# Bergvca/string_grouper

Hardware: AMD Instinct MI355X
Metric: hot-path rows/sec (the device path of match_strings: tokenise + tf-idf + postings + SpGEMM-topn, inputs resident in HBM), 663k-name self-join ntop=10 min_sim=0.8; match_strings end to end: match_strings_rows_per_s (higher is better)
Workload: dtype f32

## Files before the change

string_grouper_amd/csrc/sg_internal.h:

```cpp
#pragma once

#include <hip/hip_runtime.h>
#include <stdint.h>
#include <stdio.h>
#include <stdlib.h>
#include <string.h>

#include <map>
#include <memory>
#include <mutex>
#include <new>
#include <string>
#include <vector>

#include "../../include/sg_hip.h"

#define SG_WAVE 64
#define SG_NUM_XCD 8

void sg_set_error(const char *fmt, ...);

#define SG_HIP_TRY(expr)                                                                        \
    do {                                                                                        \
        hipError_t _e = (expr);                                                                 \
// ... 202 lines not shown
    int64_t n_orig = 0, n_u = 0;
    uint32_t *d_gid = nullptr;
    uint32_t *d_group_ptr = nullptr;
    uint32_t *d_members = nullptr;
    uint32_t *d_rep_rows = nullptr;
    int64_t *d_rep_start = nullptr;
    int32_t *d_rep_len = nullptr;
    struct sg_csr *unique = nullptr;
    const struct sg_csr *pending_src = nullptr;
};

struct sg_postings {
    sg_ctx *ctx = nullptr;
    int64_t n_right = 0, n_terms = 0, nnz = 0;
    int32_t dtype = SG_F32;
    int32_t tile_log2 = 12;
    int32_t n_tiles = 0;
    const int64_t *b_indptr = nullptr;
    const int32_t *b_indices = nullptr;
    const void *b_data = nullptr;
    uint32_t *d_seg = nullptr;
    uint32_t *d_term_len = nullptr;
    uint32_t *d_term_start = nullptr;
    int32_t *d_rows = nullptr;
    void *d_vals = nullptr;
    sg_csr src;
    int32_t split = 1;
    void *d_fwd = nullptr;
    uint32_t *d_fwd_ptr = nullptr;
    void *d_blk = nullptr;
    uint32_t blk_bytes = 0;
    void *d_q8 = nullptr;
    mutable bool q8_early = true;
    uint32_t *d_filt = nullptr;
    sg_csr *permuted = nullptr;
    uint32_t *d_orig_of = nullptr, *d_pos_of = nullptr;
    struct SgScoreCtx *d_score_ctx = nullptr;
    uint32_t *d_ends = nullptr;
    int32_t nt_pad = 0;
    int32_t fold_log2 = 0;
    uint32_t *d_ends8 = nullptr;
    int32_t nv_pad = 0;
    float norm_up = 0.f;
    uint32_t freq_min = 0;
    bool cosine_like = false;
    float max_norm2 = 0.f;
// ... 128 lines not shown
```

string_grouper_amd/csrc/sg_postings.hip:

```cpp
#include <stdlib.h>

#include <memory>
#include <optional>

#include "sg_internal.h"
#include "sg_scan.h"

__device__ __forceinline__ int64_t row_of_thread(int64_t g, int32_t tile_log2, int32_t n_tiles) {
    return ((g % n_tiles) << tile_log2) | (g / n_tiles);
}

template <typename T>
__global__ void __launch_bounds__(256) postings_count(const int64_t *__restrict__ indptr,
                                                      const int32_t *__restrict__ indices, int64_t n_rows,
                                                      int32_t tile_log2, int32_t n_tiles, uint32_t *seg_counts) {
    const int64_t j = row_of_thread((int64_t)blockIdx.x * blockDim.x + threadIdx.x, tile_log2, n_tiles);
    if (j >= n_rows) return;
    const int64_t lo = indptr[j], hi = indptr[j + 1];
    const uint32_t t = (uint32_t)(j >> tile_log2);
    for (int64_t p = lo; p < hi; ++p) {
        const int64_t bin = (int64_t)indices[p] * n_tiles + t;
        atomicAdd(&seg_counts[bin], 1u);
    }
}
// ... 174 lines not shown
        if (sc_out && threadIdx.x == 0) {
            sc_out[0] = sc;
            sc.q8 = nullptr;
            sc.q8_scale = 0.f;
            sc_out[1] = sc;
        }
        if (null_slack && threadIdx.x < 512) null_slack[threadIdx.x] = sg_null_posting(threadIdx.x);
    }
    const int x = threadIdx.x & 63, y = threadIdx.x >> 6;
    const int64_t k0 = (int64_t)blockIdx.x * 64;
    auto S = [&](int64_t k, int64_t t) -> uint32_t {
        if (k >= n_terms) return term_start[n_terms];
        return t >= n_tiles ? term_start[k + 1] : term_start[k] + cnt[(t * split) * (int64_t)n_terms + k];
    };
    const int64_t t_lim = nt_pad > n_tiles ? nt_pad : n_tiles;
    for (int64_t tb = 0; tb < t_lim; tb += 64) {
        for (int tt = y; tt < 65; tt += 16) {
            const int64_t k = k0 + x;
            tile[x][tt] = k <= n_terms ? S(k, min(tb + tt, (int64_t)n_tiles)) : 0u;
        }
        __syncthreads();
        for (int kq = y; kq < 64; kq += 16) {
            const int64_t k = k0 + kq, t = tb + x;
            if (k < n_terms && t < n_tiles) seg[k * n_tiles + t] = tile[kq][x];
            if (k == n_terms && t == 0) seg[k * n_tiles] = tile[kq][0];
            if (ends && k <= n_terms && t < nt_pad)
                ends[k * nt_pad + t] = k == n_terms ? 0u : tile[kq][min(t, (int64_t)n_tiles - 1) + 1 - tb] << 2;
        }
        __syncthreads();
    }
    if (ends8) {
        for (int64_t i = threadIdx.x; i < (int64_t)64 * nv_pad; i += blockDim.x) {
            const int64_t k = k0 + (i & 63), v = i >> 6;
            if (k > n_terms) continue;
            ends8[k * nv_pad + v] = k == n_terms ? 0u : S(k, min((v + 1) << fold_log2, (int64_t)n_tiles)) << 2;
        }
    }
}

template <typename T>
__global__ void __launch_bounds__(1024) postings_fill_lds(const int64_t *__restrict__ indptr,
                                                          const int32_t *__restrict__ indices,
                                                          const T *__restrict__ data, int64_t n_rows, int32_t tile_log2,
                                                          int32_t n_terms, int32_t split,
                                                          const uint32_t *__restrict__ cnt ,
                                                          const uint32_t *__restrict__ term_start,
                                                          const uint8_t *__restrict__ is_frequent, int32_t *out_rows,
                                                          T *out_vals, uint32_t *out_filt, float inv_norm_up, int32_t fold_log2) {
// ... 305 lines not shown
#pragma unroll
                for (int b = 0; b < FB; ++b) {
                    const uint32_t e = e0 + (uint32_t)b * stride + (uint32_t)lane;
                    const uint64_t heads = __ballot(head[b]) & (~0ull >> (63 - lane));
                    const int src = heads ? 63 - __builtin_clzll(heads) : 0;
                    const uint32_t d = (uint32_t)__shfl((int)delta[b], src, 64);
                    if (e < tot) out_filt[d + e] = stage[e];
                }
            }
        }
        __syncthreads();
        if (!one_chunk) {
            for (uint32_t e = threadIdx.x; e < tot; e += blockDim.x) {
                const uint32_t k = (uint32_t)sterm[e];
                const uint32_t start = k == 0u ? 0u : lds_get16(lcnt, k - 1u);
                if (e == start) mine[k] += lds_get16(lcnt, k) - start;
            }
            __syncthreads();
        }
    }
}

__global__ void __launch_bounds__(256) term_len_kernel(const uint32_t *__restrict__ seg, int64_t n_terms, int32_t n_tiles,
                                                       uint32_t *__restrict__ term_len) {
    const int64_t k = (int64_t)blockIdx.x * blockDim.x + threadIdx.x;
    if (k < n_terms) term_len[k] = seg[(k + 1) * n_tiles] - seg[k * n_tiles];
}

template <typename T>
__global__ void __launch_bounds__(256) fwd_pack(const int64_t *__restrict__ indptr, const int32_t *__restrict__ indices,
                                                const T *__restrict__ data, int64_t n_rows, int64_t nnz,
                                                const uint32_t *__restrict__ orig_of ,
                                                uint32_t *__restrict__ fwd_ptr , void *__restrict__ fwd) {
    const int64_t i = (int64_t)blockIdx.x * blockDim.x + threadIdx.x;
    const int64_t base = indptr[0];
    if (i <= n_rows)
        reinterpret_cast<uint2 *>(fwd_ptr)[i] = make_uint2((uint32_t)(indptr[i] - base), i < n_rows ? (orig_of ? orig_of[i] : (uint32_t)i) : 0u);
    if (i >= nnz || fwd == nullptr) return;
    const int64_t p = base + i;
    if (sizeof(T) == 4) {
        reinterpret_cast<int2 *>(fwd)[i] = make_int2(indices[p], __float_as_int((float)data[p]));
    } else {
        const long long bits = __double_as_longlong((double)data[p]);
        reinterpret_cast<int4 *>(fwd)[i] = make_int4(indices[p], 0, (int)(bits & 0xffffffffll), (int)(bits >> 32));
    }
}

template <typename T>
__global__ void __launch_bounds__(256) row_blocks_kernel(const int64_t *__restrict__ indptr, const int32_t *__restrict__ indices,
// ... 315 lines not shown

static uint32_t q8_rest_unknown(const sg_ctx *ctx) { return ctx->opt_is("SG_Q8_EARLY", '0') ? ~0u : 0u; }
int sg_postings_sync_q8_early(sg_ctx *ctx, const sg_postings *Bt) {
    const bool want = q8_rest_unknown(ctx) == 0u;
    if (!Bt->d_q8 || Bt->q8_early == want || Bt->n_right <= 0) return SG_OK;
    hipLaunchKernelGGL(q8_rest_kernel, dim3((unsigned)((Bt->n_right + 255) / 256)), dim3(256), 0, ctx->stream, (uint4 *)Bt->d_q8,
                       Bt->n_right, want ? 0u : ~0u);
    if (hipGetLastError() != hipSuccess) return SG_ERR_HIP;
    Bt->q8_early = want;
    return SG_OK;
}

static size_t lds_counter_bytes(int64_t n_cols) { return (size_t)n_cols * 4 + ((size_t)(n_cols + 31) / 32) * 4; }

struct BuildPlan {
    bool cosine_like = false;
    float max_norm2 = 0.f;
    int32_t tile_cols = 0, tile_log2 = 0;
    int64_t n_tiles = 0, n_bins = 0;
    bool want_pruned = false, will_filter = false, want_q8 = false, want_blk = false;
    bool permute = false;
    bool early_rows = false;
    bool lds_path = false, lazy_full = false;
    int32_t fold_log2 = 0, nt_pad = 0, nv_pad = 0;
    float norm_up = 0.f;
    uint32_t freq_min = 0;
    bool staged = false;
    int32_t chunk_rows = 0;
    uint32_t stage_cap = 0;
    uint32_t stage_alloc = 0;
    size_t staged_lds = 0;
    int32_t split = 1;
};

struct SplitCost {
    int32_t split = 1;
    int64_t parts = 0, part_rows = 0, chunks = 0, fill_rounds = 0;
    double fill_us = 0, table_us = 0, total_us = 0;
};
static constexpr double SG_SPLIT_US_PER_TERM_AND_CHUNK = 0.78e-3, SG_SPLIT_US_PER_POSTING = 2.9e-3, SG_SPLIT_US_PER_POSTING_RECOUNT = 0.53e-3,
                        SG_SPLIT_US_PER_CELL = 3.7e-6;
static constexpr int32_t SG_SPLIT_MAX = 16, SG_SPLIT_MIN_PART_ROWS = 512;
static SplitCost split_cost(int32_t split, int32_t tile_log2, int64_t n_tiles, int64_t n_terms, double mean_nnz, int32_t chunk_rows,
                            int32_t num_cu) {
    SplitCost c;
    c.split = split;
// ... 59 lines not shown
    pl.n_tiles = B->n_rows == 0 ? 1 : ((B->n_rows + tile_cols - 1) >> pl.tile_log2);
    pl.n_bins = B->n_cols * pl.n_tiles;
    if (pl.n_bins + 1 >= (int64_t)1 << 31) {
        sg_set_error("segment table of %lld x %lld entries is too large; use more right-hand blocks",
                     (long long)B->n_cols, (long long)pl.n_tiles);
        return SG_ERR_OVERFLOW;
    }
    pl.norm_up = __builtin_nextafterf(sqrtf(max_norm2) * 1.000001f, 2.f);
    const bool q8_forced = ctx->opt_is("SG_Q8", '1');
    pl.want_q8 = pl.want_pruned && !(flags & SG_POSTINGS_TILE_FORM) && B->n_cols < ((int64_t)1 << 24) && !ctx->opt_is("SG_Q8", '0') &&
                 (q8_forced || (double)B->nnz <= 45.0 * (double)B->n_rows) &&
                 (ctx->total_mem == 0 || (size_t)SG_Q8_STRIDE * ((size_t)B->n_rows + 1) < ctx->total_mem / 16);
    pl.will_filter = pl.want_pruned && sg_pruned_supports_tile(pl.tile_log2) &&
                     (B->n_cols + 1) * ((pl.n_tiles + 3) & ~(int64_t)3) < ((int64_t)1 << 30);
    pl.want_blk = ctx->opt_is("SG_ROW_BLOCKS", '1');
    pl.permute = !(flags & SG_POSTINGS_NO_PERMUTATION);
    pl.early_rows = pl.will_filter && !pl.want_blk && pl.permute && B->n_rows > 0;
    pl.lds_path = B->n_rows > 0 && lds_counter_bytes(B->n_cols) <= 124 * 1024 && B->n_cols > 0;
    if (const char *e = ctx->opt("SG_POSTINGS_LDS")) pl.lds_path = pl.lds_path && e[0] != '0';
    pl.lazy_full = pl.will_filter && pl.lds_path && !ctx->opt_is("SG_POSTINGS_LAZY", '0');
    if (pl.will_filter) {
        pl.nt_pad = (int32_t)((pl.n_tiles + 3) & ~(int64_t)3);
        if (pl.tile_log2 == 12 && !ctx->opt_is("SG_K4_STREAM", '0')) pl.fold_log2 = 3;
        if (pl.fold_log2 > 0) {
            const int64_t n_super = (pl.n_tiles + ((int64_t)1 << pl.fold_log2) - 1) >> pl.fold_log2;
            pl.nv_pad = (int32_t)((n_super + 3) & ~(int64_t)3);
        }
        double frac = 0.005;
        if (const char *v = ctx->opt("SG_PRUNE_FREQ")) frac = atof(v);
        const double fm = frac * (double)B->n_rows;
        pl.freq_min = fm < 1.0 ? 1u : (uint32_t)fm;
    }
    if (pl.lds_path) {
        pl.staged = pl.lazy_full && !ctx->opt_is("SG_FILL_STAGED", '0') && B->n_cols <= 65535;
        const double mean_nnz = B->n_rows > 0 ? (double)B->nnz / (double)B->n_rows : 1.0;
        if (pl.staged) {
            const size_t fixed0 = ((((size_t)B->n_cols + 1) / 2 + 3) & ~(size_t)3) * 4 + (((size_t)B->n_cols + 31) / 32) * 4 + 32 * 4;
            const size_t room = fixed0 + 16384 < 158 * 1024 ? 158 * 1024 - fixed0 : 0;
            const double per_row = (mean_nnz * 1.2 > 1.0 ? mean_nnz * 1.2 : 1.0) * 6.0 + 4.0;
            const double fit = ((double)room - 64.0 * 6.0 - 32.0) / per_row;
            pl.chunk_rows = fit >= 2048.0 ? 2048 : (fit > 0.0 ? (int32_t)fit & ~63 : 0);
            pl.staged = pl.chunk_rows >= 64;
            const size_t rowp_bytes = (size_t)staged_rowp_words(pl.chunk_rows) * 4;
            pl.stage_alloc = pl.staged ? (uint32_t)((room - rowp_bytes) / 6) & ~1u : 0u;
            if (pl.stage_alloc > 65534u) pl.stage_alloc = 65534u;
            pl.stage_cap = pl.stage_alloc;
// ... 113 lines not shown
        *out = (uint32_t)need;
    return SG_OK;
}

static int alloc_index(sg_ctx *ctx, sg_postings *p, const sg_csr *B_in, const sg_csr *B, const BuildPlan &plan, int32_t flags,
                       Scratch &early, EarlyRows *rows) {
    p->n_right = B->n_rows;
    p->n_terms = B->n_cols;
    p->nnz = B->nnz;
    p->dtype = B->dtype;
    p->tile_log2 = plan.tile_log2;
    p->tile_form = (flags & SG_POSTINGS_TILE_FORM) != 0;
    p->built_from = csr_view(*B_in);
    p->built_from_valid = true;
    p->n_tiles = (int32_t)plan.n_tiles;
    p->b_indptr = B_in->d_indptr;
    p->b_indices = B_in->d_indices;
    p->b_data = B_in->d_data;
    p->cosine_like = plan.cosine_like;
    p->max_norm2 = plan.max_norm2;
    p->src = csr_view(*B);
    p->split = plan.split;
    const size_t vs = 8;
    SG_TRY(sg_alloc(ctx, (size_t)plan.n_bins + 1, &p->d_seg));
    SG_TRY(sg_alloc(ctx, (size_t)B->n_cols + 1, &p->d_term_len));
    if (!plan.lazy_full && B->dtype == SG_F64) SG_TRY(sg_alloc(ctx, (size_t)B->nnz + 64, &p->d_rows));
    if (!plan.lazy_full) SG_TRY(ctx->alloc(((size_t)B->nnz + 64) * vs, &p->d_vals));
    if (!plan.will_filter) return SG_OK;
    if (plan.want_blk) {
        SG_TRY(row_block_bytes(ctx, B, &p->blk_bytes));
        if (p->blk_bytes) SG_TRY(ctx->alloc((size_t)p->blk_bytes * ((size_t)B->n_rows + 1), &p->d_blk));
    }
    p->q8_early = q8_rest_unknown(ctx) == 0u;
    if (rows->written) {
        p->d_fwd = early.keep(rows->fwd);
        p->d_fwd_ptr = early.keep(rows->fwd_ptr);
        p->d_q8 = early.keep(rows->q8);
    } else {
        if (!p->d_blk) SG_TRY(ctx->alloc(((size_t)B->nnz + 8) * (B->dtype == SG_F64 ? 16 : 8), &p->d_fwd));
        SG_TRY(sg_alloc(ctx, 2 * ((size_t)B->n_rows + 2), &p->d_fwd_ptr));
        if (plan.want_q8 && !p->d_blk) SG_TRY(ctx->alloc((size_t)SG_Q8_STRIDE * ((size_t)B->n_rows + 1), &p->d_q8));
    }
    SG_TRY(sg_alloc(ctx, (size_t)B->nnz + 512, &p->d_filt));
    p->nt_pad = plan.nt_pad;
    SG_TRY(sg_alloc(ctx, (size_t)(B->n_cols + 1) * (size_t)p->nt_pad + 4, &p->d_ends));
    p->fold_log2 = plan.fold_log2;
    p->nv_pad = plan.nv_pad;
// ... 24 lines not shown
        SG_TRY(by_dtype(B->dtype, [&](auto tag) -> int {
            using T = decltype(tag);
            constexpr auto kern = postings_fill_lds<T>;
            SG_TRY(allow_dynamic_lds<kern>(124 * 1024));
            hipLaunchKernelGGL(kern, dim3(wgs), dim3(1024), lds, ctx->stream, B->d_indptr, B->d_indices,
                               (const T *)B->d_data, B->n_rows, p->tile_log2, (int32_t)B->n_cols, split, (const uint32_t *)cnt,
                               (const uint32_t *)p->d_term_start, (const uint8_t *)is_frequent, p->d_rows, (T *)p->d_vals, filt,
                               inv_norm, fold_log2);
            return SG_OK;
        }));
    return hipGetLastError() == hipSuccess ? SG_OK : SG_ERR_HIP;
}

static int fill_lds_path(sg_ctx *ctx, sg_postings *p, const BuildPlan &plan) {
    const sg_csr *B = &p->src;
    const unsigned wgs = (unsigned)((int64_t)p->n_tiles * plan.split);
    Scratch scratch(ctx);
    uint32_t *cnt = nullptr, *cnt16 = nullptr;
    uint8_t *is_frequent = nullptr;
    SG_TRY(scratch.alloc((size_t)((int64_t)p->n_tiles * plan.split * B->n_cols) + 1, &cnt));
    if (plan.staged) SG_TRY(scratch.alloc((size_t)((int64_t)p->n_tiles * plan.split * ((B->n_cols + 1) / 2)) + 1, &cnt16));
    SG_TRY(scratch.alloc((size_t)B->n_cols + 4, &is_frequent));
    SG_TRY(sg_alloc(ctx, (size_t)B->n_cols + 2, &p->d_term_start));
    SG_TRY(lds_count_scan_fill(ctx, p, cnt, cnt16, p->d_term_len, is_frequent, false, !plan.staged));
    if (p->d_fwd_ptr) SG_TRY(ctx->alloc(256, (void **)&p->d_score_ctx));
    hipLaunchKernelGGL(postings_tables_kernel, dim3((unsigned)((B->n_cols + 64) / 64)), dim3(1024), 0, ctx->stream, (const uint32_t *)cnt,
                       (const uint32_t *)p->d_term_start, (int32_t)B->n_cols, p->n_tiles, plan.split, p->d_seg, p->d_ends,
                       p->nt_pad, p->d_ends8, p->nv_pad, p->fold_log2, score_ctx_of(p), p->d_score_ctx,
                       p->d_filt ? p->d_filt + B->nnz : (uint32_t *)nullptr);
    if (plan.staged)
        SG_TRY(by_dtype(B->dtype, [&](auto tag) -> int {
            using T = decltype(tag);
            constexpr auto kern = postings_fill_staged<T>;
            SG_TRY(allow_dynamic_lds<kern>(160 * 1024));
            hipLaunchKernelGGL(kern, dim3(wgs), dim3(1024), plan.staged_lds, ctx->stream, B->d_indptr,
                               B->d_indices, (const T *)B->d_data, B->n_rows, p->tile_log2, (int32_t)B->n_cols, plan.split,
                               plan.chunk_rows, plan.stage_cap, plan.stage_alloc, cnt, (const uint32_t *)cnt16,
                               (const uint32_t *)p->d_term_start, (const uint8_t *)is_frequent,
                               p->d_filt, 1.0f / p->norm_up, p->fold_log2);
            return SG_OK;
        }));
    return hipGetLastError() == hipSuccess ? SG_OK : SG_ERR_HIP;
}

static int fill_global_path(sg_ctx *ctx, sg_postings *p, const BuildPlan &plan) {
    const sg_csr *B = &p->src;
// ... 9 lines not shown
        by_dtype(B->dtype, [&](auto tag) {
            using T = decltype(tag);
            hipLaunchKernelGGL(postings_count<T>, dim3(grid), dim3(256), 0, ctx->stream, B->d_indptr, B->d_indices, B->n_rows,
                               p->tile_log2, p->n_tiles, p->d_seg);
            return SG_OK;
        });
        SG_HIP_TRY(hipGetLastError());
    }
    SG_TRY(sg_exclusive_scan_u32(ctx, p->d_seg, p->d_seg, n_bins, p->d_seg + n_bins));
    if (grid > 0) {
        by_dtype(B->dtype, [&](auto tag) {
            using T = decltype(tag);
            hipLaunchKernelGGL(postings_fill<T>, dim3(grid), dim3(256), 0, ctx->stream, B->d_indptr, B->d_indices,
                               (const T *)B->d_data, B->n_rows, p->tile_log2, p->n_tiles, p->d_seg, cursor, p->d_rows,
                               (T *)p->d_vals, p->d_filt, p->freq_min, inv_norm, p->fold_log2);
            return SG_OK;
        });
        if (hipGetLastError() != hipSuccess) return SG_ERR_HIP;
    }
    return SG_OK;
}

static int tables_from_seg(sg_ctx *ctx, sg_postings *p) {
    if (p->n_terms <= 0) return SG_OK;
    hipLaunchKernelGGL(term_len_kernel, dim3((unsigned)((p->n_terms + 255) / 256)), dim3(256), 0, ctx->stream,
                       (const uint32_t *)p->d_seg, p->n_terms, p->n_tiles, p->d_term_len);
    if (p->d_ends || p->d_ends8)
        hipLaunchKernelGGL(ends_from_seg_kernel, dim3((unsigned)((p->n_terms + 256) / 256)), dim3(256), 0, ctx->stream,
                           (const uint32_t *)p->d_seg, p->n_terms, p->n_tiles, p->d_ends, p->nt_pad, p->d_ends8, p->nv_pad,
                           p->fold_log2);
    return hipGetLastError() == hipSuccess ? SG_OK : SG_ERR_HIP;
}

static int pack_rows(sg_ctx *ctx, sg_postings *p, bool rows_written) {
    const sg_csr *B = &p->src;
    if (p->d_fwd && !rows_written) {
        const size_t es = B->dtype == SG_F64 ? 16 : 8;
        if (hipMemsetAsync((char *)p->d_fwd + (size_t)B->nnz * es, 0, 8 * es, ctx->stream) != hipSuccess) return SG_ERR_HIP;
    }
    if (p->d_blk && B->n_rows > 0) {
        const int64_t work = B->n_rows * (int64_t)(p->blk_bytes / 16);
        const unsigned g3 = (unsigned)((work + 255) / 256);
        by_dtype(B->dtype, [&](auto tag) {
            using T = decltype(tag);
            hipLaunchKernelGGL(row_blocks_kernel<T>, dim3(g3), dim3(256), 0, ctx->stream, B->d_indptr, B->d_indices,
                               (const T *)B->d_data, B->n_rows, (const uint32_t *)p->d_orig_of, p->blk_bytes, p->d_blk);
            return SG_OK;
        });
        if (hipGetLastError() != hipSuccess) return SG_ERR_HIP;
    }
// ... 92 lines not shown
    }
    if (col) {
        p->collapse = col;
        p->caller_b_copy = csr_view(*B_in);
        p->caller_b = &p->caller_b_copy;
        p->n_right_caller = B_in->n_rows;
    }
    if (group) {
        p->build_tile_cols = tile_cols;
        p->build_flags = col ? flags : flags & 0xff;
    }
    *out = p;
    return SG_OK;
}

int sg_postings_ensure_full(sg_ctx *ctx, const sg_postings *cp) {
    sg_postings *p = const_cast<sg_postings *>(cp);
    if (p->d_vals || p->nnz <= 0) return SG_OK;
    const sg_csr *B = &p->src;
    Scratch scratch(ctx);
    uint32_t *cnt = nullptr, *len_scratch = nullptr;
    if (B->dtype == SG_F64) SG_TRY(scratch.alloc((size_t)B->nnz + 64, &p->d_rows));
    int st = scratch.alloc_bytes(((size_t)B->nnz + 64) * 8, &p->d_vals);
    if (st == SG_OK && !p->d_term_start) {
        sg_set_error("postings were built without the LDS path: nothing is lazy there");
        st = SG_ERR_BADARG;
    }
    const int32_t split = p->split > 0 ? p->split : 1;
    if (st == SG_OK) st = scratch.alloc((size_t)((int64_t)p->n_tiles * split * B->n_cols) + 1, &cnt);
    if (st == SG_OK) st = scratch.alloc((size_t)B->n_cols + 2, &len_scratch);
    if (st == SG_OK) st = lds_count_scan_fill(ctx, p, cnt, nullptr, len_scratch, nullptr, true, true);
    if (st != SG_OK) {
        p->d_vals = nullptr;
        p->d_rows = nullptr;
        return st;
    }
    scratch.keep(p->d_rows);
    scratch.keep(p->d_vals);
    return SG_OK;
}

extern "C" int sg_postings_free(sg_postings *p) {
    if (!p) return SG_OK;
    p->ctx->release(p->d_seg);
    p->ctx->release(p->d_term_len);
    p->ctx->release(p->d_term_start);
    p->ctx->release(p->d_rows);
    p->ctx->release(p->d_vals);
    p->ctx->release(p->d_fwd);
    p->ctx->release(p->d_blk);
    p->ctx->release(p->d_q8);
    p->ctx->release(p->d_fwd_ptr);
    p->ctx->release(p->d_filt);
    p->ctx->release(p->d_ends);
    p->ctx->release(p->d_ends8);
    p->ctx->release(p->d_score_ctx);
    p->ctx->release(p->d_orig_of);
    p->ctx->release(p->d_pos_of);
    sg_csr_free(p->permuted);
// ... 8 lines not shown
```

string_grouper_amd/csrc/sg_spgemm_pruned.hip:

```cpp
#define SG_WATCH_NAME sg_debug_watch_pruned
#include "sg_k4_device.h"

#ifdef SG_DEBUG_WAVE_TIMES
__device__ unsigned long long sg_debug_wave_times[4 * 16384];
extern "C" int sg_debug_read_wave_times(unsigned long long *out, int clear) {
    if (hipMemcpyFromSymbol(out, HIP_SYMBOL(sg_debug_wave_times), sizeof(sg_debug_wave_times)) != hipSuccess) return 1;
    if (clear) {
        static unsigned long long zero[4 * 16384];
        if (hipMemcpyToSymbol(HIP_SYMBOL(sg_debug_wave_times), zero, sizeof(zero)) != hipSuccess) return 1;
    }
    return 0;
}
#endif

#ifndef SG_F64_STREAM_WAVES
#define SG_F64_STREAM_WAVES 4
#endif
#define SG_SCHED_FENCE() __builtin_amdgcn_sched_barrier(0)
#define SG_ROW_PARTS_LOG2 6
#define SG_ROW_PARTS 64u
#define SG_SURV_CAP 128

__device__ __forceinline__ uint64_t ballot64(bool p) { return __builtin_amdgcn_ballot_w64(p); }

// ... 482 lines not shown
                pv.d_chunk_count[pos >> 9] = pos & 511u;
                atomicAdd(pv.d_totals, (unsigned long long)(pos & 511u));
            }
            ch = atomicAdd(pv.d_chunks_used, 1u);
        }
        pos = (uint32_t)__builtin_amdgcn_readfirstlane((int)ch) << 9;
    }
    if ((pos >> 9) < pair_chunks) {
        if (lane < cnt) {
            const size_t o = (size_t)(pos >> 9) * SG_PAIR_CHUNK + (pos & 511u) + (uint32_t)lane;
            pv.d_i[o] = (uint32_t)c;
            pv.d_j[o] = row_out;
            reinterpret_cast<T *>(pv.d_s)[o] = s;
        }
        if (lane == 0) atomicAdd(&pv.d_row_count[row_out], (uint32_t)cnt);
    }
    __builtin_amdgcn_wave_barrier();
    if (lane == 0) surv[SG_SURV_CAP - 1] = (int)(pos + (uint32_t)cnt);
}

template <typename T, int TILE_LOG2, bool SYM, bool WIDE, int FOLD_LOG2, bool SHARE = false>
__global__ void __launch_bounds__(64, (sizeof(T) == 8 && FOLD_LOG2 > 0) ? SG_F64_STREAM_WAVES : 4)
spgemm_topn_pruned_kernel(const int64_t *__restrict__ a_indptr, const int32_t *__restrict__ a_indices,
                          const T *__restrict__ a_data, uint32_t n_left, const uint32_t *__restrict__ seg,
                          const uint32_t *__restrict__ ends, int32_t nt_pad, uint32_t n_terms,
                          const uint32_t *__restrict__ filt, int32_t n_tiles,
                          const SgScoreCtx *__restrict__ sc ,
                          int32_t keep, int32_t out_stride, T thr,
                          float s_budget , float norm_b ,
                          uint32_t freq_min ,
                          int32_t *__restrict__ out_cols, T *__restrict__ out_vals, int32_t *__restrict__ out_cnt,
                          uint32_t *row_counter, uint32_t *flagged_count, uint32_t *flagged_rows,
                          unsigned long long *stats ,
                          const SgPairSink *__restrict__ pairs ,
                          uint32_t pair_chunks ,
                          uint32_t sym_lo, uint32_t sym_hi ,
                          const uint32_t *__restrict__ row_list , const uint32_t *row_list_len,
                          const uint32_t *__restrict__ ends8 , int32_t nv_pad,
                          uint32_t null_off ,
                          uint32_t n_right ,
                          uint32_t *heavy_count, uint32_t *heavy_rows ,
                          uint32_t sym_step, uint32_t deal_floor ,
                          uint32_t part_cfg ) {
    constexpr int TILE = 1 << TILE_LOG2;
    constexpr int SLOTS = WIDE ? 2 : 1;
    constexpr int AB = TILE_LOG2 + 1;
    constexpr uint32_t ADDR_MASK = ((1u << AB) - 1u) & ~3u;
// ... 54 lines not shown
            if (orig_of) row_out = (uint32_t)__builtin_amdgcn_readfirstlane((int)orig_of[row]);
        }
        const int64_t rlo = a_indptr[row];
        const int nnz = __builtin_amdgcn_readfirstlane((int)(a_indptr[row + 1] - rlo));
        if (nnz > 64 * SLOTS) {
            if (lane == 0) flagged_rows[atomicAdd(flagged_count, 1u)] = row;
            continue;
        }
        if (nnz == 0) continue;
        int k[SLOTS];
        T a[SLOTS], a2[SLOTS];
        uint32_t df[SLOTS], lo_e[SLOTS], key[SLOTS];
        float w[SLOTS], cum[SLOTS];
        uint64_t fm[SLOTS];
#pragma unroll
        for (int sl = 0; sl < SLOTS; ++sl) {
            k[sl] = 0;
            a[sl] = (T)0;
            df[sl] = lo_e[sl] = 0;
            const bool have = lane + 64 * sl < nnz;
            if (have) {
                k[sl] = a_indices[rlo + lane + 64 * sl];
                a[sl] = a_data[rlo + lane + 64 * sl];
                const uint32_t *sp = seg + (int64_t)k[sl] * n_tiles;
                lo_e[sl] = sp[0];
                df[sl] = sp[n_tiles] - lo_e[sl];
            }
            a2[sl] = mul_rn<T>(a[sl], a[sl]);
            w[sl] = have ? (sizeof(T) == 4 ? (float)a2[sl] : (float)a[sl] * (float)a[sl]) * 1.00001f : 0.f;
            cum[sl] = 0.f;
            key[sl] = (min(df[sl], (1u << 25) - 1u) << 7) | (127u - (uint32_t)(lane + 64 * sl));
            fm[sl] = ballot64(have && df[sl] >= freq_min);
        }
        const bool sum_own = SYM && FOLD_LOG2 > 0 && !part_mode;
        T own = (T)0;
        auto rank_step = [&](int sl_q, int f) {
            const uint32_t kq = wave_read<uint32_t>(key[sl_q], f);
            const float wq = wave_read<float>(w[sl_q], f);
#pragma unroll
            for (int sl = 0; sl < SLOTS; ++sl) cum[sl] += kq >= key[sl] ? wq : 0.f;
        };
        if (sum_own) {
#pragma unroll
            for (int sl_q = 0; sl_q < SLOTS; ++sl_q) {
                const int n_q = min(nnz - 64 * sl_q, 64);
                for (int f = 0; f < n_q; ++f) {
                    own = add_rn<T>(own, wave_read<T>(a2[sl_q], f));
                    if ((fm[sl_q] >> f) & 1ull) rank_step(sl_q, f);
                }
// ... 1004 lines not shown
    uint32_t part_cfg = 0;
};

struct RowList {
    uint32_t *base = nullptr;
    uint32_t *count() const { return base; }
    uint32_t *counter() const { return base ? base + 1 : nullptr; }
    uint32_t *rows() const { return base ? base + 4 : nullptr; }
};

template <typename T, int TILE_LOG2, bool SYM, bool WIDE, int FOLD_LOG2>
static int launch_pruned(const PrunedJob &job, const PrunedLaunch &l) {
    sg_ctx *ctx = job.ctx;
    const sg_csr *A = job.A;
    const sg_postings *Bt = job.Bt;
    const sg_topn *r = job.r;
    const PairList &pl = *job.pl;
    const T thr = (T)job.threshold;
    const size_t lds = pruned_lds(TILE_LOG2, FOLD_LOG2, A->dtype);
    unsigned grid = pruned_grid(ctx, TILE_LOG2, SYM ? (int64_t)pl.rows() : A->n_rows, FOLD_LOG2, A->dtype);
    if (WIDE && grid > (unsigned)ctx->num_cu * 4u && (double)A->nnz <= 48.0 * (double)A->n_rows) grid = (unsigned)ctx->num_cu * 4u;
    constexpr bool SPLITS = SYM && !WIDE && FOLD_LOG2 > 0;
    const bool share = SPLITS && (l.heavy_count != nullptr || l.part_cfg != 0u);
    if (sg_q8_applies(ctx, Bt, (double)thr)) SG_TRY(sg_postings_sync_q8_early(ctx, Bt));
    auto kernel = share ? spgemm_topn_pruned_kernel<T, TILE_LOG2, SYM, WIDE, FOLD_LOG2, SPLITS>
                        : spgemm_topn_pruned_kernel<T, TILE_LOG2, SYM, WIDE, FOLD_LOG2, false>;
    hipLaunchKernelGGL(kernel, dim3(grid), dim3(64), lds, ctx->stream, A->d_indptr,
                       A->d_indices, (const T *)A->d_data, (uint32_t)A->n_rows, (const uint32_t *)Bt->d_seg,
                       (const uint32_t *)Bt->d_ends, Bt->nt_pad, (uint32_t)Bt->n_terms,
                       (const uint32_t *)Bt->d_filt, Bt->n_tiles,
                       (const SgScoreCtx *)Bt->d_score_ctx + (sg_q8_applies(ctx, Bt, (double)thr) ? 0 : 1), job.keep, r->stride, thr,
                       job.s_budget, Bt->norm_up, Bt->freq_min, r->d_cols,
                       (T *)r->d_vals,
                       r->d_counts, l.row_counter, l.out_count, l.out_rows, job.stats, pl.d_sink, pl.sink.chunks, pl.row_lo, pl.row_hi,
                       l.in_rows, l.in_len, (const uint32_t *)Bt->d_ends8, Bt->nv_pad, (uint32_t)(Bt->nnz * 4), (uint32_t)Bt->n_right,
                       l.heavy_count, l.heavy_rows, pl.row_step, ctx->opt_is("SG_DEAL", 'f') ? 1u : 0u, l.part_cfg);
    SG_HIP_TRY(hipGetLastError());
    return SG_OK;
}

static uint32_t heavy_part_cfg(const sg_ctx *ctx, const sg_csr *A, const PairList &range, int32_t tile_log2, int32_t fold_log2) {
    uint32_t heavy_rounds = 0;
    if ((range.row_lo > 0 || (int64_t)range.row_hi < A->n_rows || range.row_step > 1) && 2 * (int64_t)range.rows() < A->n_rows) {
        const double n_idx = (double)A->n_rows;
        const double rows_per_wave = (double)range.rows() / (double)pruned_grid(ctx, tile_log2, (int64_t)range.rows(), fold_log2, A->dtype);
        const double rounds_per_row = 2.0 * 7.2e-5 * n_idx * (0.5 * ((double)range.row_lo + (double)range.row_hi) / n_idx);
        const double share = ctx->opt_double("SG_HEAVY_SHARE", 0.0);
        const double bar_share = share > 0.0 ? share : 0.05;
        const double bar = bar_share * rows_per_wave * rounds_per_row;
        heavy_rounds = bar < 128.0 ? 128u : (bar > 1.0e9 ? 1000000000u : (uint32_t)bar);
    }
    heavy_rounds = (uint32_t)ctx->opt_int("SG_HEAVY_ROUNDS", (int)heavy_rounds) & 0x7fffffffu;
// ... 347 lines not shown
```

string_grouper_amd/csrc/sg_spgemm_topn.hip:

```cpp
#include <cstring>
#include <math.h>

#include <memory>

#include "sg_internal.h"

#include "sg_k4_device.h"
#include "sg_plan.h"

static_assert(SG_PLAN_LANES == SG_TOPN_LANES, "sg_plan.h counts passes and register lists in the kernels' lanes");

typedef float f32x4 __attribute__((ext_vector_type(4)));
typedef double f64x2 __attribute__((ext_vector_type(2)));
template <typename T, typename V>
__device__ __forceinline__ bool any_above(const V &v, T thr);
template <>
__device__ __forceinline__ bool any_above<float, f32x4>(const f32x4 &v, float thr) {
    const uint32_t a = __float_as_uint(v[0]), b = __float_as_uint(v[1]), c = __float_as_uint(v[2]),
                   d = __float_as_uint(v[3]);
    const uint32_t ab = a > b ? a : b, cd = c > d ? c : d;
    return (ab > cd ? ab : cd) > __float_as_uint(thr);
}
template <>
__device__ __forceinline__ bool any_above<double, f64x2>(const f64x2 &v, double thr) {
// ... 365 lines not shown
                                                       const uint32_t *__restrict__ term_len,
                                                       int64_t *__restrict__ out_cost) {
    const int64_t i = (int64_t)blockIdx.x * blockDim.x + threadIdx.x;
    if (i >= n_left) return;
    int64_t c = 0;
    for (int64_t p = a_indptr[i]; p < a_indptr[i + 1]; ++p) c += term_len[a_indices[p]];
    out_cost[i] = c;
}

__global__ void __launch_bounds__(256) sum_counts_kernel(const int32_t *__restrict__ cnt, int64_t n,
                                                         unsigned long long *out) {
    unsigned long long local = 0;
    for (int64_t i = (int64_t)blockIdx.x * blockDim.x + threadIdx.x; i < n; i += (int64_t)gridDim.x * blockDim.x)
        local += (unsigned long long)cnt[i];
    block_add_u64(local, out);
}

template <typename T, int TILE_LOG2>
static int launch_spgemm(sg_ctx *ctx, const sg_csr *A, const sg_postings *Bt, int32_t tile_begin, int32_t tile_end,
                         int32_t keep, int32_t pass_off, sg_topn *r, T thr, uint32_t *counter, unsigned grid,
                         const uint32_t *row_list, const uint32_t *row_list_len) {
    const size_t lds = sizeof(T) << TILE_LOG2;
    constexpr auto kern = spgemm_topn_kernel<T, TILE_LOG2, 8>;
    SG_TRY(allow_dynamic_lds<kern>(lds));
    hipLaunchKernelGGL(kern, dim3(grid), dim3(64), lds, ctx->stream, A->d_indptr, A->d_indices, (const T *)A->d_data,
                       (uint32_t)A->n_rows, (const uint32_t *)Bt->d_seg, (const int32_t *)Bt->d_rows,
                       (const T *)Bt->d_vals, Bt->n_tiles, tile_begin, tile_end, keep, pass_off, r->stride, thr,
                       r->d_cols, (T *)r->d_vals, r->d_counts, counter, row_list, row_list_len, (const uint32_t *)Bt->d_orig_of);
    SG_HIP_TRY(hipGetLastError());
    return SG_OK;
}

template <typename T>
static int dispatch_spgemm(sg_ctx *ctx, const sg_csr *A, const sg_postings *Bt, int32_t tile_begin, int32_t tile_end,
                           int32_t keep, int32_t pass_off, sg_topn *r, T thr, uint32_t *counter, unsigned grid,
                           const uint32_t *row_list = nullptr, const uint32_t *row_list_len = nullptr) {
    switch (Bt->tile_log2) {
        case 10: return launch_spgemm<T, 10>(ctx, A, Bt, tile_begin, tile_end, keep, pass_off, r, thr, counter, grid, row_list, row_list_len);
        case 11: return launch_spgemm<T, 11>(ctx, A, Bt, tile_begin, tile_end, keep, pass_off, r, thr, counter, grid, row_list, row_list_len);
        case 12: return launch_spgemm<T, 12>(ctx, A, Bt, tile_begin, tile_end, keep, pass_off, r, thr, counter, grid, row_list, row_list_len);
        case 13: return launch_spgemm<T, 13>(ctx, A, Bt, tile_begin, tile_end, keep, pass_off, r, thr, counter, grid, row_list, row_list_len);
        default:
            sg_set_error("postings tile of 2^%d columns is not supported by the multiply (2^10..2^13)", Bt->tile_log2);
            return SG_ERR_UNSUPPORTED;
    }
}

unsigned sg_spgemm_exact_selfjoin_grid(const sg_ctx *ctx, const sg_postings *Bt) {
    if (!Bt) return (unsigned)ctx->num_cu * 2u;
    return (unsigned)ctx->num_cu * (unsigned)sg_plan_waves_per_cu(ctx->lds_per_cu, Bt->dtype == SG_F64, Bt->tile_log2);
}

template <typename T, int TILE_LOG2>
static int launch_selfjoin_rows(sg_ctx *ctx, const sg_csr *A, const sg_postings *Bt, int32_t keep, sg_topn *r, T thr,
                                uint32_t *row_counter, const uint32_t *row_list, const uint32_t *row_list_len,
                                const SgPairSink &sink, bool all_rows) {
    const size_t lds = sizeof(T) << TILE_LOG2;
    constexpr auto kern = spgemm_topn_selfjoin_rows_kernel<T, TILE_LOG2, 8>;
    SG_TRY(allow_dynamic_lds<kern>(lds));
    hipLaunchKernelGGL(kern, dim3(sg_spgemm_exact_selfjoin_grid(ctx, all_rows ? Bt : nullptr)), dim3(64), lds, ctx->stream, A->d_indptr, A->d_indices,
                       (const T *)A->d_data, (const uint32_t *)Bt->d_seg, (const int32_t *)Bt->d_rows, (const T *)Bt->d_vals,
                       Bt->n_tiles, keep, r->stride, thr, r->d_cols, (T *)r->d_vals, r->d_counts, row_counter, row_list,
                       row_list_len, sink, (const uint32_t *)Bt->d_orig_of);
    SG_HIP_TRY(hipGetLastError());
    return SG_OK;
}

template <typename T>
static int dispatch_selfjoin_rows(sg_ctx *ctx, const sg_csr *A, const sg_postings *Bt, int32_t keep, sg_topn *r, T thr,
                                  uint32_t *row_counter, const uint32_t *row_list, const uint32_t *row_list_len,
                                  const SgPairSink &sink, bool all_rows) {
    switch (Bt->tile_log2) {
        case 10: return launch_selfjoin_rows<T, 10>(ctx, A, Bt, keep, r, thr, row_counter, row_list, row_list_len, sink, all_rows);
        case 11: return launch_selfjoin_rows<T, 11>(ctx, A, Bt, keep, r, thr, row_counter, row_list, row_list_len, sink, all_rows);
        case 12: return launch_selfjoin_rows<T, 12>(ctx, A, Bt, keep, r, thr, row_counter, row_list, row_list_len, sink, all_rows);
        case 13: return launch_selfjoin_rows<T, 13>(ctx, A, Bt, keep, r, thr, row_counter, row_list, row_list_len, sink, all_rows);
        default:
            sg_set_error("postings tile of 2^%d columns is not supported by the self-join form (2^10..2^13)", Bt->tile_log2);
            return SG_ERR_UNSUPPORTED;
    }
}
// ... 467 lines not shown
    if (st != SG_OK || !done) return st;
    *out = r.release();
    *applicable = 1;
    return SG_OK;
}

extern "C" int sg_selfjoin_merge(sg_ctx *ctx, sg_topn *res, const sg_postings *Bt, const int32_t *d_pairs, int64_t n_pairs,
                                 int32_t pair_words, int64_t row_lo, int64_t row_hi, int64_t row_step) {
    SG_REQUIRE(ctx && res, "null argument");
    SG_REQUIRE(n_pairs == 0 || d_pairs != nullptr, "pairs are null");
    SG_REQUIRE(pair_words == (res->dtype == SG_F64 ? 4 : 3), "pair records do not match the result's value type");
    SG_REQUIRE(row_lo >= 0 && row_lo <= row_hi && row_hi <= res->n_rows, "row range outside the result");
    SgTimer timer(ctx, SG_K_ZIP);
    return sg_selfjoin_merge_pairs(ctx, res, d_pairs, n_pairs, row_lo, row_hi, Bt ? (const uint32_t *)Bt->d_pos_of : nullptr, row_step);
}

extern "C" int sg_postings_bytes(const sg_postings *Bt, int64_t *pruned_multiply_bytes) {
    SG_REQUIRE(Bt && pruned_multiply_bytes, "null argument");
    int64_t b = 0;
    if (Bt->d_filt) {
        const int64_t es = Bt->dtype == SG_F64 ? 16 : 8;
        b += 4 * (Bt->nnz + 512);
        b += 4 * (Bt->n_terms + 1) * (int64_t)(Bt->fold_log2 > 0 ? Bt->nv_pad : Bt->nt_pad);
        if (Bt->d_fwd) b += es * (Bt->nnz + 8);
        if (Bt->d_fwd_ptr) b += 8 * (Bt->n_right + 2);
        if (Bt->d_blk) b += (int64_t)Bt->blk_bytes * (Bt->n_right + 1);
        if (Bt->d_q8) b += 16 * (Bt->n_right + 1) + 4 * Bt->nnz + 8 * Bt->n_right;
    }
    *pruned_multiply_bytes = b;
    return SG_OK;
}

extern "C" int sg_postings_rows(const sg_postings *Bt, int64_t *n_index_rows, int64_t *n_caller_rows,
                                const uint32_t **d_group_of_row) {
    SG_REQUIRE(Bt != nullptr, "postings are null");
    if (n_index_rows) *n_index_rows = Bt->n_right;
    if (n_caller_rows) *n_caller_rows = Bt->collapse ? Bt->collapse->n_orig : Bt->n_right;
    if (d_group_of_row) *d_group_of_row = Bt->collapse ? Bt->collapse->d_gid : nullptr;
    return SG_OK;
}

extern "C" int sg_topn_expand_groups(sg_ctx *ctx, const sg_postings *Bt, const sg_topn *groups, const int32_t *d_rows,
                                     int64_t n_rows, sg_topn **out) {
    SG_REQUIRE(ctx && Bt && groups && out, "null argument");
    SG_REQUIRE(Bt->collapse != nullptr, "the index was not built over groups of identical rows (sg_postings_rows)");
    const SgCollapse *c = Bt->collapse;
// ... 130 lines not shown
```

Before: 110.8 million.

## Defer the per-tile segment table when folded pruning runs on the lazy LDS path

When the index is built on the lazy LDS path with folded super-tiles, the full n_terms×n_tiles segment table is no longer allocated or written at build time. The pruned kernel now reads each term's list bounds from the compact per-term start array instead. The segment table is produced later in ensure_full, only when the exact kernels need it. This cuts the build's memory writes and footprint, at the cost of more bookkeeping (the lds_built flag) and new guard checks.

```diff
diff --git a/string_grouper_amd/csrc/sg_internal.h b/string_grouper_amd/csrc/sg_internal.h
--- a/string_grouper_amd/csrc/sg_internal.h
+++ b/string_grouper_amd/csrc/sg_internal.h
@@ -248,6 +248,7 @@
     uint32_t *d_seg = nullptr;
     uint32_t *d_term_len = nullptr;
     uint32_t *d_term_start = nullptr;
+    bool lds_built = false;
     int32_t *d_rows = nullptr;
     void *d_vals = nullptr;
     sg_csr src;
diff --git a/string_grouper_amd/csrc/sg_postings.hip b/string_grouper_amd/csrc/sg_postings.hip
--- a/string_grouper_amd/csrc/sg_postings.hip
+++ b/string_grouper_amd/csrc/sg_postings.hip
@@ -220,8 +220,8 @@
         __syncthreads();
         for (int kq = y; kq < 64; kq += 16) {
             const int64_t k = k0 + kq, t = tb + x;
-            if (k < n_terms && t < n_tiles) seg[k * n_tiles + t] = tile[kq][x];
-            if (k == n_terms && t == 0) seg[k * n_tiles] = tile[kq][0];
+            if (seg && k < n_terms && t < n_tiles) seg[k * n_tiles + t] = tile[kq][x];
+            if (seg && k == n_terms && t == 0) seg[k * n_tiles] = tile[kq][0];
             if (ends && k <= n_terms && t < nt_pad)
                 ends[k * nt_pad + t] = k == n_terms ? 0u : tile[kq][min(t, (int64_t)n_tiles - 1) + 1 - tb] << 2;
         }
@@ -573,9 +573,10 @@
 }
 
 __global__ void __launch_bounds__(256) term_len_kernel(const uint32_t *__restrict__ seg, int64_t n_terms, int32_t n_tiles,
-                                                       uint32_t *__restrict__ term_len) {
+                                                       uint32_t *__restrict__ term_len, uint32_t *__restrict__ term_start) {
     const int64_t k = (int64_t)blockIdx.x * blockDim.x + threadIdx.x;
     if (k < n_terms) term_len[k] = seg[(k + 1) * n_tiles] - seg[k * n_tiles];
+    if (k <= n_terms) term_start[k] = seg[k * n_tiles];
 }
 
 template <typename T>
@@ -937,6 +938,7 @@
     bool permute = false;
     bool early_rows = false;
     bool lds_path = false, lazy_full = false;
+    bool lazy_seg = false;
     int32_t fold_log2 = 0, nt_pad = 0, nv_pad = 0;
     float norm_up = 0.f;
     uint32_t freq_min = 0;
@@ -1042,6 +1044,7 @@
     if (pl.will_filter) {
         pl.nt_pad = (int32_t)((pl.n_tiles + 3) & ~(int64_t)3);
         if (pl.tile_log2 == 12 && !ctx->opt_is("SG_K4_STREAM", '0')) pl.fold_log2 = 3;
+        pl.lazy_seg = pl.lazy_full && pl.fold_log2 > 0 && B->nnz > 0;
         if (pl.fold_log2 > 0) {
             const int64_t n_super = (pl.n_tiles + ((int64_t)1 << pl.fold_log2) - 1) >> pl.fold_log2;
             pl.nv_pad = (int32_t)((n_super + 3) & ~(int64_t)3);
@@ -1201,7 +1204,7 @@
     p->src = csr_view(*B);
     p->split = plan.split;
     const size_t vs = 8;
-    SG_TRY(sg_alloc(ctx, (size_t)plan.n_bins + 1, &p->d_seg));
+    if (!plan.lazy_seg) SG_TRY(sg_alloc(ctx, (size_t)plan.n_bins + 1, &p->d_seg));
     SG_TRY(sg_alloc(ctx, (size_t)B->n_cols + 1, &p->d_term_len));
     if (!plan.lazy_full && B->dtype == SG_F64) SG_TRY(sg_alloc(ctx, (size_t)B->nnz + 64, &p->d_rows));
     if (!plan.lazy_full) SG_TRY(ctx->alloc(((size_t)B->nnz + 64) * vs, &p->d_vals));
@@ -1272,6 +1275,7 @@
     if (plan.staged) SG_TRY(scratch.alloc((size_t)((int64_t)p->n_tiles * plan.split * ((B->n_cols + 1) / 2)) + 1, &cnt16));
     SG_TRY(scratch.alloc((size_t)B->n_cols + 4, &is_frequent));
     SG_TRY(sg_alloc(ctx, (size_t)B->n_cols + 2, &p->d_term_start));
+    p->lds_built = true;
     SG_TRY(lds_count_scan_fill(ctx, p, cnt, cnt16, p->d_term_len, is_frequent, false, !plan.staged));
     if (p->d_fwd_ptr) SG_TRY(ctx->alloc(256, (void **)&p->d_score_ctx));
     hipLaunchKernelGGL(postings_tables_kernel, dim3((unsigned)((B->n_cols + 64) / 64)), dim3(1024), 0, ctx->stream, (const uint32_t *)cnt,
@@ -1327,10 +1331,10 @@
 }
 
 static int tables_from_seg(sg_ctx *ctx, sg_postings *p) {
-    if (p->n_terms <= 0) return SG_OK;
-    hipLaunchKernelGGL(term_len_kernel, dim3((unsigned)((p->n_terms + 255) / 256)), dim3(256), 0, ctx->stream,
-                       (const uint32_t *)p->d_seg, p->n_terms, p->n_tiles, p->d_term_len);
-    if (p->d_ends || p->d_ends8)
+    SG_TRY(sg_alloc(ctx, (size_t)p->n_terms + 2, &p->d_term_start));
+    hipLaunchKernelGGL(term_len_kernel, dim3((unsigned)((p->n_terms + 256) / 256)), dim3(256), 0, ctx->stream,
+                       (const uint32_t *)p->d_seg, p->n_terms, p->n_tiles, p->d_term_len, p->d_term_start);
+    if (p->n_terms > 0 && (p->d_ends || p->d_ends8))
         hipLaunchKernelGGL(ends_from_seg_kernel, dim3((unsigned)((p->n_terms + 256) / 256)), dim3(256), 0, ctx->stream,
                            (const uint32_t *)p->d_seg, p->n_terms, p->n_tiles, p->d_ends, p->nt_pad, p->d_ends8, p->nv_pad,
                            p->fold_log2);
@@ -1469,19 +1473,28 @@
     uint32_t *cnt = nullptr, *len_scratch = nullptr;
     if (B->dtype == SG_F64) SG_TRY(scratch.alloc((size_t)B->nnz + 64, &p->d_rows));
     int st = scratch.alloc_bytes(((size_t)B->nnz + 64) * 8, &p->d_vals);
-    if (st == SG_OK && !p->d_term_start) {
+    if (st == SG_OK && !p->lds_built) {
         sg_set_error("postings were built without the LDS path: nothing is lazy there");
         st = SG_ERR_BADARG;
     }
     const int32_t split = p->split > 0 ? p->split : 1;
     if (st == SG_OK) st = scratch.alloc((size_t)((int64_t)p->n_tiles * split * B->n_cols) + 1, &cnt);
     if (st == SG_OK) st = scratch.alloc((size_t)B->n_cols + 2, &len_scratch);
+    uint32_t *seg = nullptr;
+    if (st == SG_OK && !p->d_seg) st = scratch.alloc((size_t)(p->n_terms * p->n_tiles) + 1, &seg);
     if (st == SG_OK) st = lds_count_scan_fill(ctx, p, cnt, nullptr, len_scratch, nullptr, true, true);
+    if (st == SG_OK && seg) {
+        hipLaunchKernelGGL(postings_tables_kernel, dim3((unsigned)((B->n_cols + 64) / 64)), dim3(1024), 0, ctx->stream, (const uint32_t *)cnt,
+                           (const uint32_t *)p->d_term_start, (int32_t)B->n_cols, p->n_tiles, split, seg, (uint32_t *)nullptr, 0,
+                           (uint32_t *)nullptr, 0, 0, SgScoreCtx(), (SgScoreCtx *)nullptr, (uint32_t *)nullptr);
+        if (hipGetLastError() != hipSuccess) st = SG_ERR_HIP;
+    }
     if (st != SG_OK) {
         p->d_vals = nullptr;
         p->d_rows = nullptr;
         return st;
     }
+    if (seg) p->d_seg = scratch.keep(seg);
     scratch.keep(p->d_rows);
     scratch.keep(p->d_vals);
     return SG_OK;
diff --git a/string_grouper_amd/csrc/sg_spgemm_pruned.hip b/string_grouper_amd/csrc/sg_spgemm_pruned.hip
--- a/string_grouper_amd/csrc/sg_spgemm_pruned.hip
+++ b/string_grouper_amd/csrc/sg_spgemm_pruned.hip
@@ -528,7 +528,8 @@
 template <typename T, int TILE_LOG2, bool SYM, bool WIDE, int FOLD_LOG2, bool SHARE = false>
 __global__ void __launch_bounds__(64, (sizeof(T) == 8 && FOLD_LOG2 > 0) ? SG_F64_STREAM_WAVES : 4)
 spgemm_topn_pruned_kernel(const int64_t *__restrict__ a_indptr, const int32_t *__restrict__ a_indices,
-                          const T *__restrict__ a_data, uint32_t n_left, const uint32_t *__restrict__ seg,
+                          const T *__restrict__ a_data, uint32_t n_left,
+                          const uint32_t *__restrict__ starts ,
                           const uint32_t *__restrict__ ends, int32_t nt_pad, uint32_t n_terms,
                           const uint32_t *__restrict__ filt, int32_t n_tiles,
                           const SgScoreCtx *__restrict__ sc ,
@@ -629,9 +630,9 @@
             if (have) {
                 k[sl] = a_indices[rlo + lane + 64 * sl];
                 a[sl] = a_data[rlo + lane + 64 * sl];
-                const uint32_t *sp = seg + (int64_t)k[sl] * n_tiles;
+                const uint32_t *sp = FOLD_LOG2 > 0 ? starts + k[sl] : starts + (int64_t)k[sl] * n_tiles;
                 lo_e[sl] = sp[0];
-                df[sl] = sp[n_tiles] - lo_e[sl];
+                df[sl] = sp[FOLD_LOG2 > 0 ? 1 : n_tiles] - lo_e[sl];
             }
             a2[sl] = mul_rn<T>(a[sl], a[sl]);
             w[sl] = have ? (sizeof(T) == 4 ? (float)a2[sl] : (float)a[sl] * (float)a[sl]) * 1.00001f : 0.f;
@@ -1682,12 +1683,13 @@
     if (WIDE && grid > (unsigned)ctx->num_cu * 4u && (double)A->nnz <= 48.0 * (double)A->n_rows) grid = (unsigned)ctx->num_cu * 4u;
     constexpr bool SPLITS = SYM && !WIDE && FOLD_LOG2 > 0;
     const bool share = SPLITS && (l.heavy_count != nullptr || l.part_cfg != 0u);
+    SG_REQUIRE((FOLD_LOG2 > 0 ? Bt->d_term_start : Bt->d_seg) != nullptr, "the index lacks the table of its lists' bounds");
     if (sg_q8_applies(ctx, Bt, (double)thr)) SG_TRY(sg_postings_sync_q8_early(ctx, Bt));
     auto kernel = share ? spgemm_topn_pruned_kernel<T, TILE_LOG2, SYM, WIDE, FOLD_LOG2, SPLITS>
                         : spgemm_topn_pruned_kernel<T, TILE_LOG2, SYM, WIDE, FOLD_LOG2, false>;
     hipLaunchKernelGGL(kernel, dim3(grid), dim3(64), lds, ctx->stream, A->d_indptr,
-                       A->d_indices, (const T *)A->d_data, (uint32_t)A->n_rows, (const uint32_t *)Bt->d_seg,
-                       (const uint32_t *)Bt->d_ends, Bt->nt_pad, (uint32_t)Bt->n_terms,
+                       A->d_indices, (const T *)A->d_data, (uint32_t)A->n_rows,
+                       (const uint32_t *)(FOLD_LOG2 > 0 ? Bt->d_term_start : Bt->d_seg), (const uint32_t *)Bt->d_ends, Bt->nt_pad, (uint32_t)Bt->n_terms,
                        (const uint32_t *)Bt->d_filt, Bt->n_tiles,
                        (const SgScoreCtx *)Bt->d_score_ctx + (sg_q8_applies(ctx, Bt, (double)thr) ? 0 : 1), job.keep, r->stride, thr,
                        job.s_budget, Bt->norm_up, Bt->freq_min, r->d_cols,
diff --git a/string_grouper_amd/csrc/sg_spgemm_topn.hip b/string_grouper_amd/csrc/sg_spgemm_topn.hip
--- a/string_grouper_amd/csrc/sg_spgemm_topn.hip
+++ b/string_grouper_amd/csrc/sg_spgemm_topn.hip
@@ -411,6 +411,7 @@
                          const uint32_t *row_list, const uint32_t *row_list_len) {
     const size_t lds = sizeof(T) << TILE_LOG2;
     constexpr auto kern = spgemm_topn_kernel<T, TILE_LOG2, 8>;
+    SG_REQUIRE(Bt->d_seg != nullptr, "the index has no segment table yet (sg_postings_ensure_full writes it)");
     SG_TRY(allow_dynamic_lds<kern>(lds));
     hipLaunchKernelGGL(kern, dim3(grid), dim3(64), lds, ctx->stream, A->d_indptr, A->d_indices, (const T *)A->d_data,
                        (uint32_t)A->n_rows, (const uint32_t *)Bt->d_seg, (const int32_t *)Bt->d_rows,
@@ -446,6 +447,7 @@
                                 const SgPairSink &sink, bool all_rows) {
     const size_t lds = sizeof(T) << TILE_LOG2;
     constexpr auto kern = spgemm_topn_selfjoin_rows_kernel<T, TILE_LOG2, 8>;
+    SG_REQUIRE(Bt->d_seg != nullptr, "the index has no segment table yet (sg_postings_ensure_full writes it)");
     SG_TRY(allow_dynamic_lds<kern>(lds));
     hipLaunchKernelGGL(kern, dim3(sg_spgemm_exact_selfjoin_grid(ctx, all_rows ? Bt : nullptr)), dim3(64), lds, ctx->stream, A->d_indptr, A->d_indices,
                        (const T *)A->d_data, (const uint32_t *)Bt->d_seg, (const int32_t *)Bt->d_rows, (const T *)Bt->d_vals,
@@ -959,6 +961,7 @@
         const int64_t es = Bt->dtype == SG_F64 ? 16 : 8;
         b += 4 * (Bt->nnz + 512);
         b += 4 * (Bt->n_terms + 1) * (int64_t)(Bt->fold_log2 > 0 ? Bt->nv_pad : Bt->nt_pad);
+        if (Bt->fold_log2 > 0) b += 4 * (Bt->n_terms + 1);
         if (Bt->d_fwd) b += es * (Bt->nnz + 8);
         if (Bt->d_fwd_ptr) b += 8 * (Bt->n_right + 2);
         if (Bt->d_blk) b += (int64_t)Bt->blk_bytes * (Bt->n_right + 1);
```

Result: no change. 111.1 million, median of 2 (+0.2%).
